# wen-yuan-zhang/MaterialRefGS

Measured on AMD Instinct MI355X. Metric: full-render fwd+bwd views/sec at 800x800/300k surfels; grad max-rel-err vs ref, higher is better.
Workload: dtype f32; 1 GPU; C3 shell scene through render_surfel: P=300000, 800x800, S=8 + deferred BRDF shading, fwd+bwd; P=300000, H=800, W=800, S=8, sh_degree=3, num_rendered=1153468, cameras_cycled=2, parallelism=single GPU, glue_epilogue=True

## Files before the change

### include/mrgs.h

```cpp
#ifndef MRGS_H_INCLUDED
#define MRGS_H_INCLUDED

#include <stddef.h>
#include <stdint.h>

#ifdef __cplusplus
extern "C" {
#endif

#define MRGS_MAX_FEATURES 24
#define MRGS_TILE 16
#define MRGS_NUM_OTHERS 7

enum {
    MRGS_OK = 0,
    MRGS_E_BAD_ARG = 1,
    MRGS_E_TOO_MANY_FEATURES = 2,
    MRGS_E_NEED_COLORS = 3,
    MRGS_E_HIP = 4,
    MRGS_E_WORKSPACE = 5,
    MRGS_E_UNSUPPORTED = 6,
    MRGS_E_INTERNAL = 7
};

// ... 102 lines not shown
} MrgsEnvMips;

int mrgs_envmap_lookup_forward(const MrgsEnvMips* mips, int64_t N, const float* dirs, const float* roughness, float* out, void* stream);
int mrgs_envmap_lookup_backward(const MrgsEnvMips* mips, int64_t N, const float* dirs, const float* roughness, const float* g_out,
                                float* g_dirs , float* g_roughness , void* stream);

typedef struct MrgsStridedMap { const float* ptr; int64_t stride_h, stride_w, stride_c; } MrgsStridedMap;
typedef struct MrgsShadeFrame {
    int32_t H, W;
    float Kinv[9];
    const float* R;
    const float* T;
    MrgsStridedMap albedo;
    MrgsStridedMap normal;
    MrgsStridedMap alpha;
    MrgsStridedMap refl;
    MrgsStridedMap roughness;
    const float* lut;
    int32_t lut_res;
} MrgsShadeFrame;

int mrgs_shade_specular_forward(const MrgsEnvMips* mips, const MrgsShadeFrame* frame, float* specular, float* direct_light,
                                float* specular_weight, void* stream);
int mrgs_shade_specular_forward_composite(const MrgsEnvMips* mips, const MrgsShadeFrame* frame, const float* base_color, const float* bg,
                                          int32_t srgb, float* specular, float* direct_light, float* specular_weight, float* render,
                                          float* diffuse, float* zero_fill, int64_t zero_floats, void* stream);
int mrgs_shade_specular_backward(const MrgsEnvMips* mips, const MrgsShadeFrame* frame, const float* g_specular, const float* g_direct_light,
                                 const float* g_specular_weight, float* g_albedo, float* g_normal, float* g_alpha, float* g_refl,
                                 float* g_roughness, void* stream);
int mrgs_surfel_shade_composite_backward(const MrgsEnvMips* mips, const MrgsShadeFrame* frame, int32_t srgb, const float* base_color,
                                         const float* specular, const float* bg, const float* g_render, const float* g_diffuse,
                                         const float* g_specular_extra, const float* g_direct_light, const float* g_specular_weight,
                                         float* g_base, float* g_normal, float* g_features, float* g_alpha, void* stream);

int mrgs_cubemap_filter_count(int32_t res, int32_t kind, float roughness, float cos_cutoff, uint32_t* row_count, float* row_wsum, void* stream);
int mrgs_cubemap_filter_fill(int32_t res, int32_t kind, float roughness, float cos_cutoff, const uint32_t* row_ptr, const float* row_wsum,
                             uint32_t* col, float* val, void* stream);
int mrgs_csr_spmv3(int32_t nrows, const uint32_t* row_ptr, const void* col, int32_t col_bytes, const void* val, int32_t val_bytes,
                   const float* row_scale, const float* x, float* y, int32_t lanes_per_row, void* stream);
#define MRGS_SPMV_MAX_BATCH 8
#define MRGS_SPMV_MAX_PANEL 1024
typedef struct MrgsSpmvDesc {
    int32_t nrows, lanes_per_row, col_bytes, val_bytes;
    const uint32_t* row_ptr;
    const void* col;
    const void* val;
    const float* row_scale;
    const float* x;
    float* y;
    const int32_t* image_rows;
    const float* pre_scale;
    const uint32_t* tile_ptr;
    const uint32_t* panel_ptr;
    const uint16_t* panel_src;
    int32_t res, n_tiles;
    int32_t max_panel, reserved;
} MrgsSpmvDesc;
int mrgs_csr_spmv3_batched(const MrgsSpmvDesc* descs, int32_t n, void* stream);
int mrgs_cube_symmetry_rows(int32_t res, int32_t* rows);
int mrgs_cubemap_mip_chain_forward(int32_t res_in, int32_t n_steps, const float* in, float* const* outs, void* stream);
int mrgs_cubemap_mip_chain_backward(int32_t res0, int32_t n_levels, float* const* g, void* stream);
int mrgs_cubemap_mip_forward(int32_t res_out, const float* in, float* out, void* stream);
int mrgs_cubemap_mip_backward(int32_t res_fine, const float* dout, float* g_fine, void* stream);

int mrgs_cubemap_encode_forward(const float* inputs, const float* cubemap, const float* fail_value, float* outputs, int32_t interp,
                                int32_t seamless, int64_t B, int32_t C, int32_t L, void* stream);
// ... 343 lines not shown
```

### materialrefgs_amd/_lib.py

```python
import ctypes
import os
import subprocess

import torch

_CSRC = os.path.join(os.path.dirname(os.path.abspath(__file__)), "csrc")
LIB_PATH = os.environ.get("MRGS_LIB") or os.path.join(_CSRC, "libmrgs.so")

c_int32, c_int64, c_float, c_void_p, c_size_t = ctypes.c_int32, ctypes.c_int64, ctypes.c_float, ctypes.c_void_p, ctypes.c_size_t


class _Sized(ctypes.Structure):

    def __init__(self, *args, **kw):
        super().__init__(ctypes.sizeof(type(self)), *args, **kw)


class MrgsRasterConfig(_Sized):
    _fields_ = [("struct_size", ctypes.c_uint32), ("P", c_int32), ("S", c_int32), ("D", c_int32), ("M", c_int32), ("H", c_int32), ("W", c_int32),
                ("tanfovx", c_float), ("tanfovy", c_float), ("scale_modifier", c_float), ("prefiltered", c_int32),
                ("debug", c_int32)]


class MrgsRasterInputs(_Sized):
# ... 259 lines not shown
                                             c_void_p, c_void_p]),
    "mrgs_densify_emit": (ctypes.c_int, [ctypes.POINTER(MrgsDensifyConfig), c_void_p, ctypes.POINTER(c_int64),
                                         ctypes.POINTER(MrgsDensifyTensor), c_int32, ctypes.c_uint64, c_void_p, c_void_p]),
    "mrgs_densify_stats": (ctypes.c_int, [c_int64, c_void_p, c_void_p, c_void_p, c_void_p, c_void_p, c_void_p, c_void_p]),
    "mrgs_env_densify_ws_bytes": (c_size_t, [c_int64]),
    "mrgs_env_densify_classify": (ctypes.c_int, [ctypes.POINTER(MrgsEnvDensifyConfig), c_void_p, c_void_p, c_void_p, c_void_p, c_void_p, c_void_p,
                                                 c_void_p, c_size_t, c_void_p, c_void_p]),
    "mrgs_env_densify_emit": (ctypes.c_int, [ctypes.POINTER(MrgsEnvDensifyConfig), c_void_p, c_int64, ctypes.POINTER(MrgsDensifyTensor), c_int32,
                                             ctypes.c_uint64, c_void_p, c_void_p, c_void_p]),
    "mrgs_env_select_ws_bytes": (c_size_t, []),
    "mrgs_env_select": (ctypes.c_int, [c_int64, c_void_p, c_int64, c_void_p, c_size_t, c_void_p, c_void_p]),
    "mrgs_env_densify_stats": (ctypes.c_int, [c_int64, c_void_p, c_void_p, c_void_p, c_void_p, c_void_p, c_void_p, c_void_p]),
    "mrgs_tsdf_fuse": (ctypes.c_int, [ctypes.POINTER(MrgsTsdfConfig), c_void_p, c_void_p, c_void_p, c_void_p]),
    "mrgs_mesh_ws_bytes": (c_size_t, [ctypes.POINTER(MrgsMeshConfig)]),
    "mrgs_mesh_count": (ctypes.c_int, [ctypes.POINTER(MrgsMeshConfig), c_void_p, c_void_p, c_size_t, c_void_p, c_void_p]),
    "mrgs_mesh_emit": (ctypes.c_int, [ctypes.POINTER(MrgsMeshConfig), c_void_p, c_void_p, c_size_t, ctypes.POINTER(c_int64), c_void_p, c_void_p,
                                      c_void_p]),
    "mrgs_mesh_clusters": (ctypes.c_int, [c_int64, c_int64, c_void_p, c_void_p, c_void_p, c_void_p]),
    "mrgs_mesh_select": (ctypes.c_int, [c_int64, c_int64, c_void_p, c_void_p, c_void_p, c_int32, c_void_p, c_void_p, c_void_p]),
    "mrgs_mesh_reindex": (ctypes.c_int, [c_int64, c_int64, c_void_p, c_void_p, c_int64, c_void_p, c_void_p]),
    "mrgs_knn_ws_bytes": (c_size_t, [c_int64]),
    "mrgs_knn_mean_dist2": (ctypes.c_int, [c_void_p, c_int64, c_void_p, c_void_p, c_size_t, c_void_p]),
    "mrgs_mark_visible": (ctypes.c_int, [c_int32, c_void_p, c_void_p, c_void_p, c_void_p, c_void_p]),
    "mrgs_envmap_lookup_forward": (ctypes.c_int, [ctypes.POINTER(MrgsEnvMips), c_int64, c_void_p, c_void_p, c_void_p, c_void_p]),
    "mrgs_envmap_lookup_backward": (ctypes.c_int, [ctypes.POINTER(MrgsEnvMips), c_int64, c_void_p, c_void_p, c_void_p, c_void_p, c_void_p,
                                                   c_void_p]),
    "mrgs_shade_specular_forward": (ctypes.c_int, [ctypes.POINTER(MrgsEnvMips), ctypes.POINTER(MrgsShadeFrame), c_void_p, c_void_p,
                                                   c_void_p, c_void_p]),
    "mrgs_shade_specular_forward_composite": (ctypes.c_int, [ctypes.POINTER(MrgsEnvMips), ctypes.POINTER(MrgsShadeFrame), c_void_p, c_void_p, c_int32,
                                                             c_void_p, c_void_p, c_void_p, c_void_p, c_void_p, c_void_p, c_int64, c_void_p]),
    "mrgs_shade_specular_backward": (ctypes.c_int, [ctypes.POINTER(MrgsEnvMips), ctypes.POINTER(MrgsShadeFrame), c_void_p, c_void_p,
                                                    c_void_p, c_void_p, c_void_p, c_void_p, c_void_p, c_void_p, c_void_p]),
    "mrgs_surfel_shade_composite_backward": (ctypes.c_int, [ctypes.POINTER(MrgsEnvMips), ctypes.POINTER(MrgsShadeFrame), c_int32] + [c_void_p] * 13),
    "mrgs_debug_export": (ctypes.c_int, [ctypes.POINTER(MrgsRasterConfig), c_void_p, c_void_p, c_void_p, c_int64, c_int32, c_void_p,
                                         c_void_p]),
    "mrgs_set_profiling": (ctypes.c_int, [c_int32]),
    "mrgs_get_kernel_times": (ctypes.c_int, [ctypes.POINTER(MrgsKernelTimes)]),
    "mrgs_strerror": (ctypes.c_char_p, [ctypes.c_int]),
    "mrgs_last_hip_error": (ctypes.c_char_p, []),
    "mrgs_version": (ctypes.c_char_p, []),
    "mrgs_abi_version": (c_int32, []),
}
MRGS_ABI_VERSION = 10

_lib = None


def build(force=False):
    if force:
        subprocess.check_call(["make", "-C", _CSRC, "-s", "clean"])
    subprocess.check_call(["make", "-C", _CSRC, "-s", "-j8"])
    return LIB_PATH


def lib():
    global _lib
    if _lib is None:
        if not os.path.exists(LIB_PATH):
            raise ImportError(
                f"{LIB_PATH} is missing: the HIP extension has not been built (run `python -c 'import __graft_entry__ as g; "
                "g.build()'` or `make -C materialrefgs_amd/csrc`). There is no CPU fallback for the rasterizer.")
        L = ctypes.CDLL(LIB_PATH)
        for name, (res, args) in SYMBOLS.items():
            fn = getattr(L, name)
            fn.restype = res
            fn.argtypes = args
# ... 52 lines not shown
```

### materialrefgs_amd/csrc/mrgs_shade.hip

```cpp
#include "mrgs_internal.h"
#include "mrgs_model_math.h"
#include "mrgs_wave.h"

struct EnvMips {
    int n;
    int res[MRGS_MAX_MIPS];
    const float* tex[MRGS_MAX_MIPS];
    float* grad[MRGS_MAX_MIPS];
    int copies[MRGS_MAX_MIPS];
    int lds_off[MRGS_MAX_MIPS];
    float min_roughness, max_roughness;
};

struct Map {
    const float* p;
    long long sh, sw, sc;
};
struct MapOut {
    float* p;
    long long sh, sw, sc;
};

__device__ __forceinline__ float shade_rcp(float x) { return __builtin_amdgcn_rcpf(x); }

// ... 490 lines not shown
    const ShadeCamS cs = shade_cam_load(cam);
    const ShadeIn in = shade_load(x, y, albedo, normal, alpha, refl, rough);
    ShadePix p;
    shade_setup(cs, x, y, in, lut, lres, p);
    const FaceUV fu = dir_to_face(p.rn);
    float dl;
    const float level = mip_level(m, p.rough, dl);
    EnvSample s;
    Taps tp[2];
    env_fetch(m, fu, level, true, s, tp);
    const size_t HW = (size_t)H * W, pix = (size_t)y * W + x;
#pragma unroll
    for (int c = 0; c < 3; c++) {
        const float light = sigmoid_fast(s.L[c]);
        const float wgt = (0.04f * (1.f - p.refl) + p.albedo[c] * p.refl) * p.fg[0] + p.fg[1];
        direct[c * HW + pix] = light;
        weight[pix * 3 + c] = wgt;
        const float spec = light * p.alpha * wgt;
        specular[c * HW + pix] = spec;
        if (render != nullptr) {
            const float d = (1.0f - p.refl) * base[c * HW + pix];
            float v = d + spec;
            if (srgb) v = lin2srgb(v);
            render[c * HW + pix] = v + bg[c] * (1.0f - p.alpha);
            diffuse[c * HW + pix] = d;
        }
    }
}

#define MRGS_SHADE_LDS_FLOATS 23552
#ifndef MRGS_SHADE_FUSED_THREADS
#define MRGS_SHADE_FUSED_THREADS 768
#endif
template <bool COMPOSITE>
__global__ void __launch_bounds__(MRGS_SHADE_FUSED_THREADS) shade_fused_bwd_kernel(
    EnvMips m, ShadeCam cam, int H, int W, Map albedo, Map normal, Map alpha, Map refl, Map rough, const float* __restrict__ lut, int lres,
    const float* __restrict__ g_specular, const float* __restrict__ g_direct, const float* __restrict__ g_weight,
    float* __restrict__ g_albedo , float* __restrict__ g_normal , float* __restrict__ g_alpha ,
    float* __restrict__ g_refl , float* __restrict__ g_rough , int tiles_x, int ntiles, int lds_floats,
    float* __restrict__ g_features, const float* __restrict__ g_refl_composite, const float* __restrict__ g_alpha_composite,
    int srgb, const float* __restrict__ base, const float* __restrict__ spec_fwd, const float* __restrict__ bg,
    const float* __restrict__ g_render, const float* __restrict__ g_diffuse, float* __restrict__ g_base)
{
    __shared__ float s_grad[MRGS_SHADE_LDS_FLOATS];
    __shared__ unsigned s_keys[MRGS_SHADE_HASH_SIZE];
    __shared__ float s_vals[MRGS_SHADE_HASH_SIZE * 3];
    __shared__ unsigned s_count;
    for (int i = threadIdx.x; i < lds_floats; i += MRGS_SHADE_FUSED_THREADS) s_grad[i] = 0.f;
    for (int i = threadIdx.x; i < MRGS_SHADE_HASH_SIZE; i += MRGS_SHADE_FUSED_THREADS) { s_keys[i] = MRGS_SHADE_KEY_NONE; s_vals[3 * i] = 0.f; s_vals[3 * i + 1] = 0.f; s_vals[3 * i + 2] = 0.f; }
    if (threadIdx.x == 0) s_count = 0u;
    __syncthreads();
    const ShadeAcc A = {s_grad, s_keys, s_vals, &s_count};
    const size_t HW = (size_t)H * W;
    unsigned flushed_at = 0u;
    int since_check = 0;
    const ShadeCamS cs = shade_cam_load(cam);
    unsigned grad_mask = 0u;
#pragma unroll
    for (int i = 0; i < MRGS_MAX_MIPS; i++) grad_mask |= (i < m.n && m.grad[i] != nullptr) ? (1u << i) : 0u;
    for (int t = blockIdx.x; t < ntiles; t += gridDim.x) {
        const int x_ = (t % tiles_x) * 64 + (threadIdx.x & 63), y_ = (t / tiles_x) * (MRGS_SHADE_FUSED_THREADS / 64) + (threadIdx.x >> 6);
        const bool valid = x_ < W && y_ < H;
        const int x = min(x_, W - 1), y = min(y_, H - 1);
        const size_t pix = (size_t)y * W + x;
        const ShadeIn in = shade_load(x, y, albedo, normal, alpha, refl, rough);
        float gs_[3], gd_[3], gw_[3];
        float g_refl_c = 0.f, g_alpha_c = 0.f;
#pragma unroll
        for (int c = 0; c < 3; c++) {
            gs_[c] = (valid && g_specular) ? g_specular[c * HW + pix] : 0.f;
            gd_[c] = (valid && g_direct) ? g_direct[c * HW + pix] : 0.f;
            gw_[c] = (valid && g_weight) ? g_weight[pix * 3 + c] : 0.f;
        }
        if constexpr (COMPOSITE) {
            const float k = 1.0f - in.refl;
#pragma unroll
            for (int c = 0; c < 3; c++) {
                const float b = base[c * HW + pix];
                const float gR = (valid && g_render != nullptr) ? g_render[c * HW + pix] : 0.0f;
                g_alpha_c -= bg[c] * gR;
                float gl = gR;
                if (srgb) gl *= lin2srgb_grad(k * b + spec_fwd[c * HW + pix]);
                const float gd = gl + ((valid && g_diffuse != nullptr) ? g_diffuse[c * HW + pix] : 0.0f);
                if (valid) g_base[c * HW + pix] = k * gd;
                g_refl_c -= b * gd;
                gs_[c] += gl;
            }
        } else if (g_features != nullptr) {
            g_refl_c = g_refl_composite[pix];
            g_alpha_c = g_alpha_composite[pix];
        }
        ShadePix p;
        shade_setup(cs, x, y, in, lut, lres, p);
        const FaceUV fu = dir_to_face(p.rn);
        float dl;
        const float level = mip_level(m, p.rough, dl);
        EnvSample s;
        Taps tp[2];
        env_fetch(m, fu, level, true, s, tp);
        float gL[3], ga = 0.f, gm = 0.f, gfg0 = 0.f, gfg1 = 0.f, galb[3];
#pragma unroll
        for (int c = 0; c < 3; c++) {
            const float light = sigmoid_fast(s.L[c]);
            const float basec = 0.04f * (1.f - p.refl) + p.albedo[c] * p.refl;
            const float wgt = basec * p.fg[0] + p.fg[1];
            const float gs = gs_[c];
            const float gd = gd_[c] + gs * p.alpha * wgt;
            const float gw = gw_[c] + gs * light * p.alpha;
            ga += gs * light * wgt;
            gL[c] = gd * light * (1.f - light);
            galb[c] = gw * p.refl * p.fg[0];
            gm += gw * (p.albedo[c] - 0.04f) * p.fg[0];
            gfg0 += gw * basec;
            gfg1 += gw;
        }
        f3 g_rn;
        float g_level;
        env_fetch_bwd<false>(m, fu, p.rn, s, tp, gL, g_rn, g_level);
        const float rg = dot3(p.rn, g_rn);
        const float irl = shade_rcp(p.rlen);
        const f3 g_r = mk((g_rn.x - p.rn.x * rg) * irl, (g_rn.y - p.rn.y * rg) * irl, (g_rn.z - p.rn.z * rg) * irl);
        const float g_ndv = p.u_in ? gfg0 * p.dfg_du[0] + gfg1 * p.dfg_du[1] : 0.f;
        const float grn = dot3(g_r, p.n);
        const f3 gn = mk(2.f * p.ndv * g_r.x + (2.f * grn + g_ndv) * p.wo.x, 2.f * p.ndv * g_r.y + (2.f * grn + g_ndv) * p.wo.y,
                         2.f * p.ndv * g_r.z + (2.f * grn + g_ndv) * p.wo.z);
        const float g_rough_v = (p.v_in ? gfg0 * p.dfg_dv[0] + gfg1 * p.dfg_dv[1] : 0.f) + g_level * dl;
        if (valid) {
            g_normal[pix * 3] = gn.x; g_normal[pix * 3 + 1] = gn.y; g_normal[pix * 3 + 2] = gn.z;
            if (g_features != nullptr) {
                g_alpha[pix] = g_alpha_c + ga;
                g_features[pix] = g_refl_c + gm;
                g_features[HW + pix] = g_rough_v;
#pragma unroll
                for (int c = 0; c < 3; c++) { g_features[(2 + c) * HW + pix] = galb[c]; g_features[(5 + c) * HW + pix] = 0.0f; }
            } else {
#pragma unroll
                for (int c = 0; c < 3; c++) g_albedo[pix * 3 + c] = galb[c];
                g_alpha[pix] = ga;
                g_refl[pix] = gm;
                g_rough[pix] = g_rough_v;
            }
        }
        if (!valid) { gL[0] = 0.f; gL[1] = 0.f; gL[2] = 0.f; }
        if (grad_mask != 0u && __builtin_amdgcn_ballot_w64(gL[0] != 0.f || gL[1] != 0.f || gL[2] != 0.f) != 0ull)
            env_scatter_tile(m, grad_mask, A, s, tp, gL);
        if (++since_check < 4) continue;
        since_check = 0;
        __syncthreads();
        const unsigned taken = s_count;
        if (taken - flushed_at > MRGS_SHADE_HASH_SIZE / 2) {
            acc_flush_hash(m, A, MRGS_SHADE_FUSED_THREADS);
            flushed_at = taken;
        }
        __syncthreads();
    }
    __syncthreads();
    acc_flush_hash(m, A, MRGS_SHADE_FUSED_THREADS);
    for (int l = 0; l < m.n; l++) {
        if (m.lds_off[l] < 0 || m.grad[l] == nullptr) continue;
        const int n = 6 * m.res[l] * m.res[l] * 3;
        float* dst = m.grad[l] + (size_t)(blockIdx.x % (unsigned)m.copies[l]) * (size_t)n;
        for (int i = threadIdx.x; i < n; i += MRGS_SHADE_FUSED_THREADS) {
            const float v = s_grad[m.lds_off[l] + i];
            if (v != 0.f) atomicAdd(dst + i, v);
        }
    }
}

__device__ __forceinline__ float cm_pixel_area(int x, int y, int N)
{
    if (N <= 1) return 1.0f;
    const int H = N / 2;
    x = abs(x - H); y = abs(y - H);
    const float dx = atanf((float)(x + 1) / (float)H) - atanf((float)x / (float)H);
    const float dy = atanf((float)(y + 1) / (float)H) - atanf((float)y / (float)H);
    return dx * dy;
}
__device__ __forceinline__ f3 cm_normalize(f3 v)
// ... 471 lines not shown
                                       int64_t zero_floats, void* stream)
{
    EnvMips m;
    if (int rc = make_mips(mips, m)) return rc;
    if (!fr || fr->H <= 0 || fr->W <= 0 || !fr->R || !fr->T || !fr->lut || fr->lut_res < 1 || !specular || !direct_light || !specular_weight)
        return MRGS_E_BAD_ARG;
    if (zero_floats < 0 || (zero_floats > 0 && !zero_fill)) return MRGS_E_BAD_ARG;
    ShadeCam cam;
    for (int i = 0; i < 9; i++) cam.Kinv[i] = fr->Kinv[i];
    cam.R = fr->R; cam.T = fr->T;
    const dim3 grid((fr->W + 63) / 64, (fr->H + 3) / 4), block(256);
    hipLaunchKernelGGL(shade_specular_fwd_kernel, grid, block, 0, (hipStream_t)stream, m, cam, fr->H, fr->W, to_map(fr->albedo), to_map(fr->normal),
                       to_map(fr->alpha), to_map(fr->refl), to_map(fr->roughness), fr->lut, fr->lut_res, specular, direct_light, specular_weight,
                       base_color, bg, srgb, render, diffuse, zero_fill, (long long)zero_floats);
    return MRGS_LAUNCH_STATUS();
}

int mrgs_shade_specular_forward(const MrgsEnvMips* mips, const MrgsShadeFrame* fr, float* specular, float* direct_light, float* specular_weight,
                                void* stream)
{
    return shade_specular_forward_impl(mips, fr, specular, direct_light, specular_weight, nullptr, nullptr, 0, nullptr, nullptr, nullptr, 0, stream);
}

int mrgs_shade_specular_forward_composite(const MrgsEnvMips* mips, const MrgsShadeFrame* fr, const float* base_color, const float* bg, int32_t srgb,
                                          float* specular, float* direct_light, float* specular_weight, float* render, float* diffuse,
                                          float* zero_fill, int64_t zero_floats, void* stream)
{
    if (!base_color || !bg || !render || !diffuse) return MRGS_E_BAD_ARG;
    return shade_specular_forward_impl(mips, fr, specular, direct_light, specular_weight, base_color, bg, srgb ? 1 : 0, render, diffuse, zero_fill,
                                       zero_floats, stream);
}

struct ShadeCompositeArgs { int srgb; const float *base, *spec_fwd, *bg, *g_render, *g_diffuse; float* g_base; };

static int shade_specular_backward_impl(const MrgsEnvMips* mips, const MrgsShadeFrame* fr, const float* g_specular, const float* g_direct_light,
                                        const float* g_specular_weight, float* g_albedo, float* g_normal, float* g_alpha, float* g_refl,
                                        float* g_roughness, float* g_features, const ShadeCompositeArgs* composite, void* stream)
{
    EnvMips m;
    if (int rc = make_mips(mips, m)) return rc;
    if (!fr || fr->H <= 0 || fr->W <= 0 || !fr->R || !fr->T || !fr->lut || !g_normal || !g_alpha) return MRGS_E_BAD_ARG;
    if (composite ? (!g_features || !composite->base || !composite->spec_fwd || !composite->bg || !composite->g_base)
                  : (!g_albedo || !g_refl || !g_roughness)) return MRGS_E_BAD_ARG;
    for (int l = 0; l < m.n; l++)
        if (m.grad[l] != nullptr && 6ll * m.res[l] * m.res[l] >= (1ll << 24)) return MRGS_E_UNSUPPORTED;
    ShadeCam cam;
    for (int i = 0; i < 9; i++) cam.Kinv[i] = fr->Kinv[i];
    cam.R = fr->R; cam.T = fr->T;
    static int n_cu = 0;
    if (n_cu == 0) {
        int dev = 0, v = 0;
        if (hipGetDevice(&dev) == hipSuccess && hipDeviceGetAttribute(&v, hipDeviceAttributeMultiprocessorCount, dev) == hipSuccess && v > 0) n_cu = v;
        else n_cu = 256;
    }
    int lds_floats = 0;
    for (int l = m.n - 1; l >= 0; l--) {
        const int n = 6 * m.res[l] * m.res[l] * 3;
        if (m.grad[l] == nullptr || lds_floats + n > MRGS_SHADE_LDS_FLOATS) break;
        m.lds_off[l] = lds_floats;
        lds_floats += n;
    }
    const int rows = MRGS_SHADE_FUSED_THREADS / 64;
    const int tiles_x = (fr->W + 63) / 64, ntiles = tiles_x * ((fr->H + rows - 1) / rows);
    const dim3 grid(ntiles < n_cu ? ntiles : n_cu), block(MRGS_SHADE_FUSED_THREADS);
    if (composite)
        hipLaunchKernelGGL((shade_fused_bwd_kernel<true>), grid, block, 0, (hipStream_t)stream, m, cam, fr->H, fr->W, to_map(fr->albedo), to_map(fr->normal),
                           to_map(fr->alpha), to_map(fr->refl), to_map(fr->roughness), fr->lut, fr->lut_res, g_specular, g_direct_light, g_specular_weight,
                           g_albedo, g_normal, g_alpha, g_refl, g_roughness, tiles_x, ntiles, lds_floats, g_features, (const float*)nullptr, (const float*)nullptr,
                           composite->srgb, composite->base, composite->spec_fwd, composite->bg, composite->g_render, composite->g_diffuse, composite->g_base);
    else
        hipLaunchKernelGGL((shade_fused_bwd_kernel<false>), grid, block, 0, (hipStream_t)stream, m, cam, fr->H, fr->W, to_map(fr->albedo), to_map(fr->normal),
                           to_map(fr->alpha), to_map(fr->refl), to_map(fr->roughness), fr->lut, fr->lut_res, g_specular, g_direct_light, g_specular_weight,
                           g_albedo, g_normal, g_alpha, g_refl, g_roughness, tiles_x, ntiles, lds_floats, g_features, (const float*)nullptr, (const float*)nullptr,
                           0, (const float*)nullptr, (const float*)nullptr, (const float*)nullptr, (const float*)nullptr, (const float*)nullptr, (float*)nullptr);
    return MRGS_LAUNCH_STATUS();
}

int mrgs_shade_specular_backward(const MrgsEnvMips* mips, const MrgsShadeFrame* fr, const float* g_specular, const float* g_direct_light,
                                 const float* g_specular_weight, float* g_albedo, float* g_normal, float* g_alpha, float* g_refl,
                                 float* g_roughness, void* stream)
{
    return shade_specular_backward_impl(mips, fr, g_specular, g_direct_light, g_specular_weight, g_albedo, g_normal, g_alpha, g_refl, g_roughness,
                                        nullptr, nullptr, stream);
}

int mrgs_surfel_shade_composite_backward(const MrgsEnvMips* mips, const MrgsShadeFrame* fr, int32_t srgb, const float* base_color, const float* specular,
                                         const float* bg, const float* g_render, const float* g_diffuse, const float* g_specular_extra,
                                         const float* g_direct_light, const float* g_specular_weight, float* g_base, float* g_normal, float* g_features,
                                         float* g_alpha, void* stream)
{
    if (!g_features) return MRGS_E_BAD_ARG;
    const ShadeCompositeArgs ca = {srgb, base_color, specular, bg, g_render, g_diffuse, g_base};
    return shade_specular_backward_impl(mips, fr, g_specular_extra, g_direct_light, g_specular_weight, nullptr, g_normal, g_alpha, nullptr, nullptr,
                                        g_features, &ca, stream);
}

int mrgs_cubemap_filter_count(int32_t res, int32_t kind, float roughness, float cos_cutoff, uint32_t* row_count, float* row_wsum, void* stream)
{
    if (res < 1 || res > 1024 || (kind != 0 && kind != 1) || !row_count || !row_wsum) return MRGS_E_BAD_ARG;
    const int NT = 6 * res * res;
    hipLaunchKernelGGL(cubemap_filter_build_kernel<0>, dim3((NT + 255) / 256), dim3(256), 0, (hipStream_t)stream, res, kind, roughness, cos_cutoff,
                       row_count, row_wsum, (const uint32_t*)nullptr, (uint32_t*)nullptr, (float*)nullptr);
    return MRGS_LAUNCH_STATUS();
}

int mrgs_cubemap_filter_fill(int32_t res, int32_t kind, float roughness, float cos_cutoff, const uint32_t* row_ptr, const float* row_wsum,
                             uint32_t* col, float* val, void* stream)
{
    if (res < 1 || res > 1024 || (kind != 0 && kind != 1) || !row_ptr || !row_wsum || !col || !val) return MRGS_E_BAD_ARG;
    const int NT = 6 * res * res;
    hipLaunchKernelGGL(cubemap_filter_build_kernel<1>, dim3((NT + 255) / 256), dim3(256), 0, (hipStream_t)stream, res, kind, roughness, cos_cutoff,
                       (uint32_t*)nullptr, const_cast<float*>(row_wsum), row_ptr, col, val);
    return MRGS_LAUNCH_STATUS();
}

int mrgs_csr_spmv3(int32_t nrows, const uint32_t* row_ptr, const void* col, int32_t col_bytes, const void* val, int32_t val_bytes,
                   const float* row_scale, const float* x, float* y, int32_t lanes_per_row, void* stream)
{
    if (nrows < 1 || !row_ptr || !col || !val || !x || !y || (col_bytes != 2 && col_bytes != 4) || (val_bytes != 2 && val_bytes != 4 && val_bytes != 8)) return MRGS_E_BAD_ARG;
    if (val_bytes != 4 && !row_scale) return MRGS_E_BAD_ARG;
    hipStream_t st = (hipStream_t)stream;
    if (val_bytes == 8) {
        if (col_bytes != 2 || lanes_per_row < 64 || (nrows & 3) || ((uintptr_t)x & 15u) || ((uintptr_t)val & 7u)) return MRGS_E_BAD_ARG;
        hipLaunchKernelGGL(csr_spmv3_blk4_kernel, dim3((unsigned)(((size_t)nrows * 64 + 255) / 256)), dim3(256), 0, st, nrows, row_ptr, (const uint16_t*)col,
                           (const uint2*)val, row_scale, x, y);
        return MRGS_LAUNCH_STATUS();
    }
// ... 127 lines not shown
```

### materialrefgs_amd/shading.py

```python
import ctypes
import os

import numpy as np
import torch

from . import _lib
from ._cache import Bounded
from ._lib import MRGS_MAX_MIPS, MrgsEnvMips, MrgsShadeFrame, MrgsStridedMap
from .gs_utils import safe_normalize

_ASSETS = os.path.join(os.path.dirname(os.path.abspath(__file__)), "assets")
_FG_LUT_CACHE = {}


def load_fg_lut(device, path=None):
    key = (str(device), path)
    if key not in _FG_LUT_CACHE:
        if path is None:
            arr = np.load(os.path.join(_ASSETS, "fg_lut_256.npy"))
        else:
            arr = np.fromfile(path, dtype=np.float32).reshape(256, 256, 2)
        _FG_LUT_CACHE[key] = torch.from_numpy(np.ascontiguousarray(arr, dtype=np.float32)).to(device)
    return _FG_LUT_CACHE[key]

# ... 694 lines not shown
        H, W, dev = features.shape[1], features.shape[2], features.device
        mips = [m.detach().contiguous() for m in mips]
        R, T = R.contiguous().float(), T.contiguous().float()
        maps = _SurfelShade._maps(features, normal_map, render_alpha)
        o = dict(dtype=torch.float32, device=dev)
        specular, direct, weight = torch.empty((3, H, W), **o), torch.empty((3, H, W), **o), torch.empty((H, W, 3), **o)
        render, diffuse = torch.empty((3, H, W), **o), torch.empty((3, H, W), **o)
        fr = _ShadeSpecular._frame(H, W, Kinv, R, T, maps, lut)
        ms = _mips_struct(mips, None, min_roughness, max_roughness)
        L = _lib.lib()
        ctx.texel_grads = None
        n_fixed = 14
        if vis is None and any(ctx.needs_input_grad[n_fixed + i] for i in range(len(mips))):
            ctx.texel_grads = _grad_buffers(mips, [ctx.needs_input_grad[n_fixed + i] for i in range(len(mips))], cleared_by_caller=True)
        zf = None if ctx.texel_grads is None else ctx.texel_grads[1]
        with _lib.guard(dev):
            st = _lib.stream_ptr(dev)
            indirect_color = None
            if vis is None:
                _lib.check(L.mrgs_shade_specular_forward_composite(ctypes.byref(ms), ctypes.byref(fr), _ptr(base_color), _ptr(bg), int(bool(srgb)),
                                                                   _ptr(specular), _ptr(direct), _ptr(weight), _ptr(render), _ptr(diffuse),
                                                                   _ptr(zf), 0 if zf is None else zf.numel(), st))
            else:
                _lib.check(L.mrgs_shade_specular_forward(ctypes.byref(ms), ctypes.byref(fr), _ptr(specular), _ptr(direct), _ptr(weight), st))
            if vis is not None:
                vis = vis.detach().float().contiguous()
                indirect_color = torch.empty((3, H, W), **o)
                _lib.check(L.mrgs_indirect_blend_forward(H, W, _ptr(direct), _ptr(weight), ctypes.byref(_smap(features.permute(1, 2, 0)[:, :, 5:8], 3)),
                                                         ctypes.byref(_smap(render_alpha.permute(1, 2, 0), 1)), _ptr(vis), _ptr(specular),
                                                         _ptr(indirect_color), st))
                _lib.check(L.mrgs_surfel_composite_forward(H, W, int(bool(srgb)), _ptr(base_color), _ptr(features[0:1]), _ptr(specular),
                                                           _ptr(render_alpha), _ptr(bg), _ptr(render), _ptr(diffuse), st))
        ctx.has_vis = vis is not None
        ctx.save_for_backward(base_color, features, normal_map, render_alpha, bg, specular, lut, R, T, direct if vis is not None else None,
                              weight if vis is not None else None, vis, *mips)
        ctx.Kinv, ctx.params, ctx.srgb = Kinv, (min_roughness, max_roughness), int(bool(srgb))
        ctx.n_fixed = n_fixed
        if vis is not None:
            return render, diffuse, specular, direct, weight, indirect_color
        return render, diffuse, specular, direct, weight

    @staticmethod
    def _maps(features, normal_map, render_alpha):
        hwc = features.permute(1, 2, 0)
        return [hwc[:, :, 2:5], normal_map, render_alpha.permute(1, 2, 0), hwc[:, :, 0:1], hwc[:, :, 1:2]]

    @staticmethod
    def backward(ctx, g_render, g_diffuse, g_spec_out, g_direct, g_weight, *_g_indirect_color):
        base_color, features, normal_map, render_alpha, bg, specular, lut, R, T, direct, weight, vis, *mips = ctx.saved_tensors
        H, W, dev = features.shape[1], features.shape[2], features.device
        c = lambda g: None if g is None else g.contiguous().float()
        g_render, g_diffuse, g_spec_out, g_direct, g_weight = c(g_render), c(g_diffuse), c(g_spec_out), c(g_direct), c(g_weight)
        o = dict(dtype=torch.float32, device=dev)
        g_base = torch.empty((3, H, W), **o)
        g_normal = torch.empty((H, W, 3), **o)
        g_stack = torch.empty((8 if ctx.grad_stack is None else ctx.grad_stack.height, H, W), **o)
        g_features = g_stack[:8]
        if ctx.grad_stack is not None:
            ctx.grad_stack.stack = g_stack
        g_alpha = torch.empty((1, H, W), **o)
        needs = [ctx.needs_input_grad[ctx.n_fixed + i] for i in range(len(mips))]
        if not ctx.has_vis:
            tg, ctx.texel_grads = ctx.texel_grads, None
            if tg is not None:
                grads, grads_flat = tg
            else:
                grads, grads_flat = _grad_buffers(mips, needs, cleared_by_caller=True)
                if grads_flat is not None:
                    grads_flat.zero_()
        else:
            grads, grads_flat = _grad_buffers(mips, needs, cleared_by_caller=True)
        fr = _ShadeSpecular._frame(H, W, ctx.Kinv, R, T, _SurfelShade._maps(features, normal_map, render_alpha), lut)
        ms = _mips_struct(mips, grads, *ctx.params)
        L = _lib.lib()
        with _lib.guard(dev):
            st = _lib.stream_ptr(dev)
            if not ctx.has_vis:
                _lib.check(L.mrgs_surfel_shade_composite_backward(ctypes.byref(ms), ctypes.byref(fr), ctx.srgb, _ptr(base_color), _ptr(specular), _ptr(bg),
                                                                  _ptr(g_render), _ptr(g_diffuse), _ptr(g_spec_out), _ptr(g_direct), _ptr(g_weight),
                                                                  _ptr(g_base), _ptr(g_normal), _ptr(g_features), _ptr(g_alpha), st))
            else:
                g_spec = torch.empty((3, H, W), **o)
                g_refl_c, g_alpha_c = torch.empty((1, H, W), **o), torch.empty((1, H, W), **o)
                g_albedo = torch.empty((H, W, 3), **o)
                g_alpha_s, g_refl_s, g_rough = torch.empty((H, W, 1), **o), torch.empty((H, W, 1), **o), torch.empty((H, W, 1), **o)
                _lib.check(L.mrgs_surfel_composite_backward(H, W, ctx.srgb, _ptr(base_color), _ptr(features[0:1]), _ptr(specular), _ptr(bg),
                                                            _ptr(g_render), _ptr(g_diffuse), _ptr(g_base), _ptr(g_refl_c), _ptr(g_spec), _ptr(g_alpha_c),
                                                            _ptr(grads_flat), 0 if grads_flat is None else grads_flat.numel(), st))
                if g_spec_out is not None:
                    g_spec = g_spec + g_spec_out
                gd_b, gw_b = torch.empty((3, H, W), **o), torch.empty((H, W, 3), **o)
                g_ind, g_alpha_b = torch.empty((H, W, 3), **o), torch.empty((H, W, 1), **o)
                g_ic = c(_g_indirect_color[0]) if _g_indirect_color else None
                _lib.check(L.mrgs_indirect_blend_backward(H, W, _ptr(direct), _ptr(weight), ctypes.byref(_smap(features.permute(1, 2, 0)[:, :, 5:8], 3)),
                                                          ctypes.byref(_smap(render_alpha.permute(1, 2, 0), 1)), _ptr(vis), _ptr(g_spec), _ptr(g_ic),
                                                          _ptr(gd_b), _ptr(gw_b), _ptr(g_ind), _ptr(g_alpha_b), st))
                g_direct = gd_b if g_direct is None else g_direct + gd_b
                g_weight = gw_b if g_weight is None else g_weight + gw_b
                _lib.check(L.mrgs_shade_specular_backward(ctypes.byref(ms), ctypes.byref(fr), None, _ptr(g_direct), _ptr(g_weight), _ptr(g_albedo),
                                                          _ptr(g_normal), _ptr(g_alpha_s), _ptr(g_refl_s), _ptr(g_rough), st))
                _lib.check(L.mrgs_surfel_feature_grads(H, W, _ptr(g_refl_c), _ptr(g_refl_s), _ptr(g_rough), _ptr(g_albedo), _ptr(g_ind), _ptr(g_features),
                                                       _ptr(g_alpha_c), _ptr(g_alpha_s), _ptr(g_alpha_b), _ptr(g_alpha), st))
        return (g_base, g_features, g_normal, g_alpha, None, None, None, None, None, None, None, None, None, None, *_sum_copies(grads))


_KINV = Bounded(4096)


def _kinv_tuple(K):
    a = np.asarray(K, dtype=np.float32)
    key = a.tobytes()
    t = _KINV.get(key)
    if t is None:
# ... 68 lines not shown
```

Baseline: 1201 views/s.

## Skip env fetch in shading backward for all-background wavefronts using saved forward outputs

```diff
diff --git a/include/mrgs.h b/include/mrgs.h
--- a/include/mrgs.h
+++ b/include/mrgs.h
@@ -158,6 +158,11 @@
                                          const float* specular, const float* bg, const float* g_render, const float* g_diffuse,
                                          const float* g_specular_extra, const float* g_direct_light, const float* g_specular_weight,
                                          float* g_base, float* g_normal, float* g_features, float* g_alpha, void* stream);
+int mrgs_surfel_shade_composite_backward_reuse(const MrgsEnvMips* mips, const MrgsShadeFrame* frame, int32_t srgb, const float* base_color,
+                                               const float* specular, const float* bg, const float* g_render, const float* g_diffuse,
+                                               const float* g_specular_extra, const float* g_direct_light, const float* g_specular_weight,
+                                               float* g_base, float* g_normal, float* g_features, float* g_alpha, const float* direct_light,
+                                               const float* specular_weight, void* stream);
 
 int mrgs_cubemap_filter_count(int32_t res, int32_t kind, float roughness, float cos_cutoff, uint32_t* row_count, float* row_wsum, void* stream);
 int mrgs_cubemap_filter_fill(int32_t res, int32_t kind, float roughness, float cos_cutoff, const uint32_t* row_ptr, const float* row_wsum,
diff --git a/materialrefgs_amd/_lib.py b/materialrefgs_amd/_lib.py
--- a/materialrefgs_amd/_lib.py
+++ b/materialrefgs_amd/_lib.py
@@ -315,6 +315,8 @@
     "mrgs_shade_specular_backward": (ctypes.c_int, [ctypes.POINTER(MrgsEnvMips), ctypes.POINTER(MrgsShadeFrame), c_void_p, c_void_p,
                                                     c_void_p, c_void_p, c_void_p, c_void_p, c_void_p, c_void_p, c_void_p]),
     "mrgs_surfel_shade_composite_backward": (ctypes.c_int, [ctypes.POINTER(MrgsEnvMips), ctypes.POINTER(MrgsShadeFrame), c_int32] + [c_void_p] * 13),
+    "mrgs_surfel_shade_composite_backward_reuse": (ctypes.c_int, [ctypes.POINTER(MrgsEnvMips), ctypes.POINTER(MrgsShadeFrame), c_int32]
+                                                   + [c_void_p] * 15),
     "mrgs_debug_export": (ctypes.c_int, [ctypes.POINTER(MrgsRasterConfig), c_void_p, c_void_p, c_void_p, c_int64, c_int32, c_void_p,
                                          c_void_p]),
     "mrgs_set_profiling": (ctypes.c_int, [c_int32]),
diff --git a/materialrefgs_amd/csrc/mrgs_shade.hip b/materialrefgs_amd/csrc/mrgs_shade.hip
--- a/materialrefgs_amd/csrc/mrgs_shade.hip
+++ b/materialrefgs_amd/csrc/mrgs_shade.hip
@@ -546,6 +546,25 @@
 #ifndef MRGS_SHADE_FUSED_THREADS
 #define MRGS_SHADE_FUSED_THREADS 768
 #endif
+__device__ __forceinline__ void shade_store_background(size_t pix, size_t HW, float ga, float g_alpha_c, float g_refl_c, float* __restrict__ g_albedo,
+                                                       float* __restrict__ g_normal, float* __restrict__ g_alpha, float* __restrict__ g_refl,
+                                                       float* __restrict__ g_rough, float* __restrict__ g_features)
+{
+    g_normal[pix * 3] = 0.f; g_normal[pix * 3 + 1] = 0.f; g_normal[pix * 3 + 2] = 0.f;
+    if (g_features != nullptr) {
+        g_alpha[pix] = g_alpha_c + ga;
+        g_features[pix] = g_refl_c;
+#pragma unroll
+        for (int c = 1; c < 8; c++) g_features[c * HW + pix] = 0.0f;
+    } else {
+#pragma unroll
+        for (int c = 0; c < 3; c++) g_albedo[pix * 3 + c] = 0.f;
+        g_alpha[pix] = ga;
+        g_refl[pix] = 0.f;
+        g_rough[pix] = 0.f;
+    }
+}
+
 template <bool COMPOSITE>
 __global__ void __launch_bounds__(MRGS_SHADE_FUSED_THREADS) shade_fused_bwd_kernel(
     EnvMips m, ShadeCam cam, int H, int W, Map albedo, Map normal, Map alpha, Map refl, Map rough, const float* __restrict__ lut, int lres,
@@ -554,7 +573,8 @@
     float* __restrict__ g_refl , float* __restrict__ g_rough , int tiles_x, int ntiles, int lds_floats,
     float* __restrict__ g_features, const float* __restrict__ g_refl_composite, const float* __restrict__ g_alpha_composite,
     int srgb, const float* __restrict__ base, const float* __restrict__ spec_fwd, const float* __restrict__ bg,
-    const float* __restrict__ g_render, const float* __restrict__ g_diffuse, float* __restrict__ g_base)
+    const float* __restrict__ g_render, const float* __restrict__ g_diffuse, float* __restrict__ g_base,
+    const float* __restrict__ fwd_direct , const float* __restrict__ fwd_weight )
 {
     __shared__ float s_grad[MRGS_SHADE_LDS_FLOATS];
     __shared__ unsigned s_keys[MRGS_SHADE_HASH_SIZE];
@@ -604,60 +624,76 @@
             g_refl_c = g_refl_composite[pix];
             g_alpha_c = g_alpha_composite[pix];
         }
-        ShadePix p;
-        shade_setup(cs, x, y, in, lut, lres, p);
-        const FaceUV fu = dir_to_face(p.rn);
-        float dl;
-        const float level = mip_level(m, p.rough, dl);
-        EnvSample s;
-        Taps tp[2];
-        env_fetch(m, fu, level, true, s, tp);
-        float gL[3], ga = 0.f, gm = 0.f, gfg0 = 0.f, gfg1 = 0.f, galb[3];
-#pragma unroll
-        for (int c = 0; c < 3; c++) {
-            const float light = sigmoid_fast(s.L[c]);
-            const float basec = 0.04f * (1.f - p.refl) + p.albedo[c] * p.refl;
-            const float wgt = basec * p.fg[0] + p.fg[1];
-            const float gs = gs_[c];
-            const float gd = gd_[c] + gs * p.alpha * wgt;
-            const float gw = gw_[c] + gs * light * p.alpha;
-            ga += gs * light * wgt;
-            gL[c] = gd * light * (1.f - light);
-            galb[c] = gw * p.refl * p.fg[0];
-            gm += gw * (p.albedo[c] - 0.04f) * p.fg[0];
-            gfg0 += gw * basec;
-            gfg1 += gw;
-        }
-        f3 g_rn;
-        float g_level;
-        env_fetch_bwd<false>(m, fu, p.rn, s, tp, gL, g_rn, g_level);
-        const float rg = dot3(p.rn, g_rn);
-        const float irl = shade_rcp(p.rlen);
-        const f3 g_r = mk((g_rn.x - p.rn.x * rg) * irl, (g_rn.y - p.rn.y * rg) * irl, (g_rn.z - p.rn.z * rg) * irl);
-        const float g_ndv = p.u_in ? gfg0 * p.dfg_du[0] + gfg1 * p.dfg_du[1] : 0.f;
-        const float grn = dot3(g_r, p.n);
-        const f3 gn = mk(2.f * p.ndv * g_r.x + (2.f * grn + g_ndv) * p.wo.x, 2.f * p.ndv * g_r.y + (2.f * grn + g_ndv) * p.wo.y,
-                         2.f * p.ndv * g_r.z + (2.f * grn + g_ndv) * p.wo.z);
-        const float g_rough_v = (p.v_in ? gfg0 * p.dfg_dv[0] + gfg1 * p.dfg_dv[1] : 0.f) + g_level * dl;
-        if (valid) {
-            g_normal[pix * 3] = gn.x; g_normal[pix * 3 + 1] = gn.y; g_normal[pix * 3 + 2] = gn.z;
-            if (g_features != nullptr) {
-                g_alpha[pix] = g_alpha_c + ga;
-                g_features[pix] = g_refl_c + gm;
-                g_features[HW + pix] = g_rough_v;
-#pragma unroll
-                for (int c = 0; c < 3; c++) { g_features[(2 + c) * HW + pix] = galb[c]; g_features[(5 + c) * HW + pix] = 0.0f; }
+        const bool covered = valid && (in.alpha != 0.f || gd_[0] != 0.f || gd_[1] != 0.f || gd_[2] != 0.f || gw_[0] != 0.f || gw_[1] != 0.f || gw_[2] != 0.f);
+        const bool background = __builtin_amdgcn_ballot_w64(covered) == 0ull;
+        if (background && fwd_direct != nullptr) {
+            float ga = 0.f;
+#pragma unroll
+            for (int c = 0; c < 3; c++) ga += gs_[c] * fwd_direct[c * HW + pix] * fwd_weight[pix * 3 + c];
+            if (valid) shade_store_background(pix, HW, ga, g_alpha_c, g_refl_c, g_albedo, g_normal, g_alpha, g_refl, g_rough, g_features);
+        } else {
+            ShadePix p;
+            shade_setup(cs, x, y, in, lut, lres, p);
+            const FaceUV fu = dir_to_face(p.rn);
+            float dl;
+            const float level = mip_level(m, p.rough, dl);
+            EnvSample s;
+            Taps tp[2];
+            env_fetch(m, fu, level, true, s, tp);
+            if (background) {
+                float ga = 0.f;
+#pragma unroll
+                for (int c = 0; c < 3; c++) ga += gs_[c] * sigmoid_fast(s.L[c]) * ((0.04f * (1.f - p.refl) + p.albedo[c] * p.refl) * p.fg[0] + p.fg[1]);
+                if (valid) shade_store_background(pix, HW, ga, g_alpha_c, g_refl_c, g_albedo, g_normal, g_alpha, g_refl, g_rough, g_features);
             } else {
-#pragma unroll
-                for (int c = 0; c < 3; c++) g_albedo[pix * 3 + c] = galb[c];
-                g_alpha[pix] = ga;
-                g_refl[pix] = gm;
-                g_rough[pix] = g_rough_v;
+                float gL[3], ga = 0.f, gm = 0.f, gfg0 = 0.f, gfg1 = 0.f, galb[3];
+#pragma unroll
+                for (int c = 0; c < 3; c++) {
+                    const float light = sigmoid_fast(s.L[c]);
+                    const float basec = 0.04f * (1.f - p.refl) + p.albedo[c] * p.refl;
+                    const float wgt = basec * p.fg[0] + p.fg[1];
+                    const float gs = gs_[c];
+                    const float gd = gd_[c] + gs * p.alpha * wgt;
+                    const float gw = gw_[c] + gs * light * p.alpha;
+                    ga += gs * light * wgt;
+                    gL[c] = gd * light * (1.f - light);
+                    galb[c] = gw * p.refl * p.fg[0];
+                    gm += gw * (p.albedo[c] - 0.04f) * p.fg[0];
+                    gfg0 += gw * basec;
+                    gfg1 += gw;
+                }
+                f3 g_rn;
+                float g_level;
+                env_fetch_bwd<false>(m, fu, p.rn, s, tp, gL, g_rn, g_level);
+                const float rg = dot3(p.rn, g_rn);
+                const float irl = shade_rcp(p.rlen);
+                const f3 g_r = mk((g_rn.x - p.rn.x * rg) * irl, (g_rn.y - p.rn.y * rg) * irl, (g_rn.z - p.rn.z * rg) * irl);
+                const float g_ndv = p.u_in ? gfg0 * p.dfg_du[0] + gfg1 * p.dfg_du[1] : 0.f;
+                const float grn = dot3(g_r, p.n);
+                const f3 gn = mk(2.f * p.ndv * g_r.x + (2.f * grn + g_ndv) * p.wo.x, 2.f * p.ndv * g_r.y + (2.f * grn + g_ndv) * p.wo.y,
+                                 2.f * p.ndv * g_r.z + (2.f * grn + g_ndv) * p.wo.z);
+                const float g_rough_v = (p.v_in ? gfg0 * p.dfg_dv[0] + gfg1 * p.dfg_dv[1] : 0.f) + g_level * dl;
+                if (valid) {
+                    g_normal[pix * 3] = gn.x; g_normal[pix * 3 + 1] = gn.y; g_normal[pix * 3 + 2] = gn.z;
+                    if (g_features != nullptr) {
+                        g_alpha[pix] = g_alpha_c + ga;
+                        g_features[pix] = g_refl_c + gm;
+                        g_features[HW + pix] = g_rough_v;
+#pragma unroll
+                        for (int c = 0; c < 3; c++) { g_features[(2 + c) * HW + pix] = galb[c]; g_features[(5 + c) * HW + pix] = 0.0f; }
+                    } else {
+#pragma unroll
+                        for (int c = 0; c < 3; c++) g_albedo[pix * 3 + c] = galb[c];
+                        g_alpha[pix] = ga;
+                        g_refl[pix] = gm;
+                        g_rough[pix] = g_rough_v;
+                    }
+                }
+                if (!valid) { gL[0] = 0.f; gL[1] = 0.f; gL[2] = 0.f; }
+                if (grad_mask != 0u && __builtin_amdgcn_ballot_w64(gL[0] != 0.f || gL[1] != 0.f || gL[2] != 0.f) != 0ull)
+                    env_scatter_tile(m, grad_mask, A, s, tp, gL);
             }
         }
-        if (!valid) { gL[0] = 0.f; gL[1] = 0.f; gL[2] = 0.f; }
-        if (grad_mask != 0u && __builtin_amdgcn_ballot_w64(gL[0] != 0.f || gL[1] != 0.f || gL[2] != 0.f) != 0ull)
-            env_scatter_tile(m, grad_mask, A, s, tp, gL);
         if (++since_check < 4) continue;
         since_check = 0;
         __syncthreads();
@@ -1195,16 +1231,19 @@
 }
 
 struct ShadeCompositeArgs { int srgb; const float *base, *spec_fwd, *bg, *g_render, *g_diffuse; float* g_base; };
+struct ShadeForwardArgs { const float *direct, *weight; };
 
 static int shade_specular_backward_impl(const MrgsEnvMips* mips, const MrgsShadeFrame* fr, const float* g_specular, const float* g_direct_light,
                                         const float* g_specular_weight, float* g_albedo, float* g_normal, float* g_alpha, float* g_refl,
-                                        float* g_roughness, float* g_features, const ShadeCompositeArgs* composite, void* stream)
+                                        float* g_roughness, float* g_features, const ShadeCompositeArgs* composite, const ShadeForwardArgs& fwd,
+                                        void* stream)
 {
     EnvMips m;
     if (int rc = make_mips(mips, m)) return rc;
     if (!fr || fr->H <= 0 || fr->W <= 0 || !fr->R || !fr->T || !fr->lut || !g_normal || !g_alpha) return MRGS_E_BAD_ARG;
     if (composite ? (!g_features || !composite->base || !composite->spec_fwd || !composite->bg || !composite->g_base)
                   : (!g_albedo || !g_refl || !g_roughness)) return MRGS_E_BAD_ARG;
+    if ((fwd.direct == nullptr) != (fwd.weight == nullptr)) return MRGS_E_BAD_ARG;
     for (int l = 0; l < m.n; l++)
         if (m.grad[l] != nullptr && 6ll * m.res[l] * m.res[l] >= (1ll << 24)) return MRGS_E_UNSUPPORTED;
     ShadeCam cam;
@@ -1230,12 +1269,14 @@
         hipLaunchKernelGGL((shade_fused_bwd_kernel<true>), grid, block, 0, (hipStream_t)stream, m, cam, fr->H, fr->W, to_map(fr->albedo), to_map(fr->normal),
                            to_map(fr->alpha), to_map(fr->refl), to_map(fr->roughness), fr->lut, fr->lut_res, g_specular, g_direct_light, g_specular_weight,
                            g_albedo, g_normal, g_alpha, g_refl, g_roughness, tiles_x, ntiles, lds_floats, g_features, (const float*)nullptr, (const float*)nullptr,
-                           composite->srgb, composite->base, composite->spec_fwd, composite->bg, composite->g_render, composite->g_diffuse, composite->g_base);
+                           composite->srgb, composite->base, composite->spec_fwd, composite->bg, composite->g_render, composite->g_diffuse, composite->g_base,
+                           fwd.direct, fwd.weight);
     else
         hipLaunchKernelGGL((shade_fused_bwd_kernel<false>), grid, block, 0, (hipStream_t)stream, m, cam, fr->H, fr->W, to_map(fr->albedo), to_map(fr->normal),
                            to_map(fr->alpha), to_map(fr->refl), to_map(fr->roughness), fr->lut, fr->lut_res, g_specular, g_direct_light, g_specular_weight,
                            g_albedo, g_normal, g_alpha, g_refl, g_roughness, tiles_x, ntiles, lds_floats, g_features, (const float*)nullptr, (const float*)nullptr,
-                           0, (const float*)nullptr, (const float*)nullptr, (const float*)nullptr, (const float*)nullptr, (const float*)nullptr, (float*)nullptr);
+                           0, (const float*)nullptr, (const float*)nullptr, (const float*)nullptr, (const float*)nullptr, (const float*)nullptr, (float*)nullptr,
+                           fwd.direct, fwd.weight);
     return MRGS_LAUNCH_STATUS();
 }
 
@@ -1244,7 +1285,7 @@
                                  float* g_roughness, void* stream)
 {
     return shade_specular_backward_impl(mips, fr, g_specular, g_direct_light, g_specular_weight, g_albedo, g_normal, g_alpha, g_refl, g_roughness,
-                                        nullptr, nullptr, stream);
+                                        nullptr, nullptr, ShadeForwardArgs{nullptr, nullptr}, stream);
 }
 
 int mrgs_surfel_shade_composite_backward(const MrgsEnvMips* mips, const MrgsShadeFrame* fr, int32_t srgb, const float* base_color, const float* specular,
@@ -1252,10 +1293,20 @@
                                          const float* g_direct_light, const float* g_specular_weight, float* g_base, float* g_normal, float* g_features,
                                          float* g_alpha, void* stream)
 {
+    return mrgs_surfel_shade_composite_backward_reuse(mips, fr, srgb, base_color, specular, bg, g_render, g_diffuse, g_specular_extra, g_direct_light,
+                                                      g_specular_weight, g_base, g_normal, g_features, g_alpha, nullptr, nullptr, stream);
+}
+
+int mrgs_surfel_shade_composite_backward_reuse(const MrgsEnvMips* mips, const MrgsShadeFrame* fr, int32_t srgb, const float* base_color,
+                                               const float* specular, const float* bg, const float* g_render, const float* g_diffuse,
+                                               const float* g_specular_extra, const float* g_direct_light, const float* g_specular_weight,
+                                               float* g_base, float* g_normal, float* g_features, float* g_alpha, const float* direct_light,
+                                               const float* specular_weight, void* stream)
+{
     if (!g_features) return MRGS_E_BAD_ARG;
     const ShadeCompositeArgs ca = {srgb, base_color, specular, bg, g_render, g_diffuse, g_base};
     return shade_specular_backward_impl(mips, fr, g_specular_extra, g_direct_light, g_specular_weight, nullptr, g_normal, g_alpha, nullptr, nullptr,
-                                        g_features, &ca, stream);
+                                        g_features, &ca, ShadeForwardArgs{direct_light, specular_weight}, stream);
 }
 
 int mrgs_cubemap_filter_count(int32_t res, int32_t kind, float roughness, float cos_cutoff, uint32_t* row_count, float* row_wsum, void* stream)
diff --git a/materialrefgs_amd/shading.py b/materialrefgs_amd/shading.py
--- a/materialrefgs_amd/shading.py
+++ b/materialrefgs_amd/shading.py
@@ -750,8 +750,7 @@
                 _lib.check(L.mrgs_surfel_composite_forward(H, W, int(bool(srgb)), _ptr(base_color), _ptr(features[0:1]), _ptr(specular),
                                                            _ptr(render_alpha), _ptr(bg), _ptr(render), _ptr(diffuse), st))
         ctx.has_vis = vis is not None
-        ctx.save_for_backward(base_color, features, normal_map, render_alpha, bg, specular, lut, R, T, direct if vis is not None else None,
-                              weight if vis is not None else None, vis, *mips)
+        ctx.save_for_backward(base_color, features, normal_map, render_alpha, bg, specular, lut, R, T, direct, weight, vis, *mips)
         ctx.Kinv, ctx.params, ctx.srgb = Kinv, (min_roughness, max_roughness), int(bool(srgb))
         ctx.n_fixed = n_fixed
         if vis is not None:
@@ -794,9 +793,10 @@
         with _lib.guard(dev):
             st = _lib.stream_ptr(dev)
             if not ctx.has_vis:
-                _lib.check(L.mrgs_surfel_shade_composite_backward(ctypes.byref(ms), ctypes.byref(fr), ctx.srgb, _ptr(base_color), _ptr(specular), _ptr(bg),
-                                                                  _ptr(g_render), _ptr(g_diffuse), _ptr(g_spec_out), _ptr(g_direct), _ptr(g_weight),
-                                                                  _ptr(g_base), _ptr(g_normal), _ptr(g_features), _ptr(g_alpha), st))
+                _lib.check(L.mrgs_surfel_shade_composite_backward_reuse(ctypes.byref(ms), ctypes.byref(fr), ctx.srgb, _ptr(base_color), _ptr(specular),
+                                                                        _ptr(bg), _ptr(g_render), _ptr(g_diffuse), _ptr(g_spec_out), _ptr(g_direct),
+                                                                        _ptr(g_weight), _ptr(g_base), _ptr(g_normal), _ptr(g_features), _ptr(g_alpha),
+                                                                        _ptr(direct), _ptr(weight), st))
             else:
                 g_spec = torch.empty((3, H, W), **o)
                 g_refl_c, g_alpha_c = torch.empty((1, H, W), **o), torch.empty((1, H, W), **o)
```

New measurement: 1203 views/s, median of 2. No clear change (+0.1%).
